# sunkafei/coffeedb

Measured on AMD Instinct MI355X. Metric: sa_build_GiB_per_s, higher is better.
Workload: dtype u64

## Files before the change

### coffeedb_amd/csrc/capi.hip

```cpp
#include <dirent.h>

#include <algorithm>
#include <chrono>
#include <condition_variable>
#include <cstdlib>
#include <cstring>
#include <thread>

#include "../../include/coffeedb_gpu.h"
#include "index_impl.h"

using namespace cdb;

namespace {

double wall_ms() {
    using namespace std::chrono;
    return duration<double, std::milli>(steady_clock::now().time_since_epoch()).count();
}

void set_error(Index& ix, const char* msg) {
    std::lock_guard<std::mutex> g(ix.err_mu);
    ix.err = msg;
}
// ... 1638 lines not shown
    else if (!std::strcmp(name, "reference_compat")) ix.reference_compat = value != 0;
    else if (!std::strcmp(name, "force_doubling")) ix.force_doubling = value != 0;
    else if (!std::strcmp(name, "initial_passes")) ix.initial_passes = (int)value;
    else if (!std::strcmp(name, "sort_variant")) ix.sort_variant = (int)value;
    else if (!std::strcmp(name, "keyhist3")) ix.keyhist3 = value != 0;
    else if (!std::strcmp(name, "key_symbols")) ix.key_symbols = (int)value;
    else if (!std::strcmp(name, "msd_first")) ix.msd_first = value != 0;
    else if (!std::strcmp(name, "msd_pair")) ix.msd_pair = value != 0;
    else if (!std::strcmp(name, "overlap_paircount")) ix.overlap_paircount = value != 0;
    else if (!std::strcmp(name, "key_directory")) { ix.key_directory = value != 0; ix.h_keydir.clear(); ix.keydir_tried = false; }
    else if (!std::strcmp(name, "fuse_records")) ix.fuse_records = value != 0;
    else if (!std::strcmp(name, "sweep_records")) ix.sweep_records = value != 0;
    else if (!std::strcmp(name, "partial_symbol")) ix.partial_symbol = value != 0;
    else if (!std::strcmp(name, "group_sort")) ix.group_sort = value != 0;
    else if (!std::strcmp(name, "list_rounds")) ix.list_rounds = value != 0;
    else if (!std::strcmp(name, "fuse_pairclass")) ix.fuse_pairclass = value != 0;
    else if (!std::strcmp(name, "group_sort_cap")) ix.group_sort_cap = (int)std::max<int64_t>(1, std::min<int64_t>(value, 1 << 20));
    else if (!std::strcmp(name, "vl_keys")) ix.vl_keys = value < 0 ? 0 : (value > 56 ? 56 : (int)value);
    else if (!std::strcmp(name, "pack_sa")) ix.pack_sa = value != 0;
    else if (!std::strcmp(name, "key_cost_model")) ix.key_cost_model = value != 0;
    else if (!std::strcmp(name, "gen_prebased")) ix.gen_prebased = value != 0;
    else if (!std::strcmp(name, "pack_entries")) ix.pack_entries = value != 0;
    else if (!std::strcmp(name, "segmented_sort")) ix.segmented_sort = value != 0;
    else if (!std::strcmp(name, "fold_root")) ix.fold_root = value != 0;
    else if (!std::strcmp(name, "fold_depth1")) ix.fold_depth1 = value != 0;
    else if (!std::strcmp(name, "flags_in_last_pass")) ix.flags_in_last_pass = value != 0;
    else if (!std::strcmp(name, "search_lanes")) ix.search_lanes = (value == 1 || value == 8) ? (int)value : 0;
    else if (!std::strcmp(name, "digit_bits")) ix.digit_bits = (int)value;
    else if (!std::strcmp(name, "fuse_keygen")) ix.fuse_keygen = value != 0;
    else if (!std::strcmp(name, "force_big_path")) ix.force_big_path = value != 0;
    else if (!std::strcmp(name, "debug_fail_build")) ix.debug_fail_build = value != 0;
    else if (!std::strcmp(name, "debug_append_path")) ix.debug_append_path = value == 1 || value == 2 ? (int)value : 0;
    else if (!std::strcmp(name, "debug_no_segcap")) ix.debug_no_segcap = value != 0;
    else if (!std::strcmp(name, "debug_starve_group")) ix.debug_starve_group = (int)value;
    else if (!std::strcmp(name, "self_check")) ix.self_check = value < 0 ? 0 : value > 3 ? 3 : (int)value;
    else if (!std::strcmp(name, "premap_generation")) ix.premap_generation = value != 0;
    else if (!std::strcmp(name, "proof_cancel")) {
        if (value) proof_stop(ix);
    }
    else if (!std::strcmp(name, "debug_damage_after_build")) ix.debug_damage_after_build = value < 0 ? 0 : (uint64_t)value;
    else if (!std::strcmp(name, "debug_fail_self_check")) ix.debug_fail_self_check = value != 0;
    else if (!std::strcmp(name, "plain_tile_order")) ix.rws.plain_order = value != 0;
    else if (!std::strcmp(name, "key_coding")) ix.key_coding = (int)value;
    else if (!std::strcmp(name, "narrow_keys")) ix.narrow_keys = value != 0;
    else if (!std::strcmp(name, "single_query")) ix.use_single_query = value != 0;
    else if (!std::strcmp(name, "resident_query")) {
// ... 5 lines not shown
    }
    else if (!std::strcmp(name, "bucket_group_limit")) ix.bucket_group_limit = (uint64_t)value;
    else if (!std::strcmp(name, "query_hit_budget"))
        ix.query_hit_budget = value > 0 ? std::min<uint64_t>((uint64_t)value, 1ull << 31) : 1;
    else if (!std::strcmp(name, "coalesce_queries")) ix.coalesce_queries = value != 0;
    else if (!std::strcmp(name, "fast_search")) ix.use_fast_search = value != 0;
    else if (!std::strcmp(name, "wave_rows")) ix.use_wave_rows = value != 0;
    else if (!std::strcmp(name, "keep_keys")) ix.keep_keys = value != 0;
    else {
        set_error(ix, (std::string("unknown option: ") + name).c_str());
        return CDB_E_INVALID;
    }
    return CDB_OK;
}

int cdb_get_stat(const cdb_index* h, const char* name, double* value) {
    if (!h || !name || !value) return CDB_E_INVALID;
    const BuildStats& b = h->ix.bstats;
    const QueryStats& q = h->ix.qstats;
    struct { const char* n; double v; } tab[] = {
        {"build_ms", b.build_ms}, {"alloc_ms", b.alloc_ms}, {"free_ms", b.free_ms}, {"rounds", (double)b.rounds}, {"ext_rounds", (double)b.ext_rounds},
        {"dbl_rounds", (double)b.dbl_rounds}, {"unresolved_after_initial", (double)b.unresolved_initial},
        {"unresolved_max", (double)b.unresolved_max}, {"sort_passes", (double)b.sort_passes},
        {"sort_passes_skipped", (double)b.sort_passes_skipped}, {"isa_built", (double)b.isa_built}, {"fused_keygen", (double)b.fused_keygen}, {"dense_keys", (double)b.dense_keys}, {"key_layout", (double)b.key_layout}, {"bucketed", (double)b.bucketed}, {"bucket_groups", (double)b.bucket_groups}, {"segmented", (double)b.segmented}, {"fused_records", (double)b.fused_records}, {"sweep_records", (double)b.sweep_records}, {"vl_key_bits", (double)b.vl_key_bits}, {"partial_levels", (double)b.partial_levels}, {"list_rounds", (double)b.list_rounds}, {"pairclass_fused", (double)b.pairclass_fused}, {"group_sorts", (double)b.group_sorts}, {"group_sort_fallbacks", (double)b.group_sort_fallbacks}, {"vl_avg_len", b.vl_avg_len}, {"vl_rate", b.vl_rate}, {"vl_est_unresolved", b.vl_est_unresolved}, {"fixed_est_unresolved", b.fixed_est_unresolved}, {"gen_prebased", (double)b.gen_prebased}, {"root_folded", (double)b.root_folded}, {"flags_in_last_pass", (double)b.flags_in_last_pass}, {"msd_first", (double)b.msd_first}, {"bucket_low_digits", (double)b.bucket_low_digits}, {"key_directory_cells", h->ix.h_keydir.empty() ? 0.0 : (double)(h->ix.h_keydir.size() - 1)}, {"group_fallbacks", (double)h->ix.group_fallbacks}, {"dense_key_retries", (double)h->ix.dense_key_retries}, {"self_check_fallbacks", (double)h->ix.self_check_fallbacks}, {"sa_packed", h->ix.sa_packed ? 1.0 : 0.0}, {"sa_bytes_per_entry", h->ix.sa_packed ? 5.0 : (double)h->ix.width}, {"self_check_pairs", (double)h->ix.self_check_pairs}, {"self_check_ms", h->ix.self_check_ms}, {"self_check_coverage", h->ix.size > 1 ? (double)h->ix.self_check_pairs / (double)(h->ix.size - 1) : 0.0},
        {"order_proved", (h->ix.proof.state.load() == 2 || h->ix.proof.state.load() == 3 || (h->ix.self_check == 2 && h->ix.width != 0)) ? 1.0 : 0.0},
        {"proof_state", (double)h->ix.proof.state.load()}, {"proof_ms", h->ix.proof.ms}, {"proof_repair_ms", h->ix.proof.repair_ms},
        {"proof_pairs", (double)h->ix.proof.pairs}, {"proof_bad_pairs", (double)h->ix.proof.found[0]}, {"proof_invalid_entries", (double)h->ix.proof.found[1]}, {"proof_skipped_pairs", (double)h->ix.proof.skipped}, {"proof_mixed_pairs", (double)h->ix.proof.mixed},
        {"proof_runs", (double)h->ix.proof.runs}, {"pool_big_mallocs", (double)DevPool::get().big_mallocs()}, {"premap_ms", h->ix.proof.premap_ms}, {"premap_bytes", (double)h->ix.proof.premap_bytes},
        {"key_symbols", (double)b.key_symbols}, {"symbol_bits", (double)b.symbol_bits},
        {"alphabet", (double)b.alphabet}, {"digit_bits", (double)b.digit_bits}, {"final_depth", (double)b.final_depth}, {"compat_rotations", (double)b.compat_rotations},
        {"compat_depth", (double)b.compat_depth},
        {"host_upload_ms", h->ix.host_upload_ms}, {"host_free_ms", h->ix.host_free_ms},
        {"resident_answers", (double)h->ix.res_answers}, {"launched_answers", (double)h->ix.launched_answers}, {"resident_mode", (double)h->ix.resident_mode},
        {"cluster_table_bytes", h->ix.clu.valid ? (double)(h->ix.clu.bytes() + h->ix.idt.bytes()) : 0.0}, {"cluster_classes", (double)h->ix.clu.nclasses},
        {"cluster_prepare_ms", h->ix.clu.prepare_ms}, {"cluster_ms", h->ix.clu.last_ms}, {"cluster_resorted", h->ix.clu.resorted ? 1.0 : 0.0},
        {"removes", (double)h->ix.rm.calls}, {"remove_compactions", (double)h->ix.rm.compactions}, {"remove_rebuilds", (double)h->ix.rm.rebuilds},
        {"remove_docs", (double)h->ix.rm.docs}, {"remove_bytes", (double)h->ix.rm.bytes}, {"remove_ms", h->ix.rm.last_ms},
        {"appends", (double)h->ix.ap.calls}, {"append_merges", (double)h->ix.ap.merges}, {"append_rebuilds", (double)h->ix.ap.rebuilds},
        {"append_docs", (double)h->ix.ap.docs}, {"append_bytes", (double)h->ix.ap.bytes}, {"append_ms", h->ix.ap.last_ms},
        {"append_keys_kept", (double)h->ix.ap.keys_kept},
        {"render_ms", h->ix.rnd.last_ms}, {"render_page_bytes", (double)h->ix.rnd.page_bytes}, {"render_spans", (double)h->ix.rnd.spans},
        {"query_ms", q.query_ms}, {"query_upload_ms", q.upload_ms}, {"query_device_ms", q.device_ms}, {"query_download_ms", q.download_ms}, {"query_hits", (double)q.nhits}, {"query_rows", (double)q.nrows},
        {"query_batches", (double)q.batches}, {"query_spec_batches", (double)q.spec_batches}, {"query_spec_spills", (double)q.spec_spills},
        {"query_wave_batches", (double)q.wave_batches}, {"query_sort_batches", (double)q.sort_batches}, {"query_sort_chunks", (double)q.sort_chunks},
        {"query_empty_batches", (double)q.empty_batches},
    };
    for (auto& e : tab)
// ... 204 lines not shown
```

### coffeedb_amd/csrc/index_impl.h

```cpp
#pragma once
#include <atomic>
#include <condition_variable>
#include <mutex>
#include <thread>
#include <string>
#include <vector>

#include "../../include/coffeedb_gpu.h"
#include "common.h"
#include "radix_sort.h"

namespace cdb {

constexpr int TEXT_PAD = 128;

struct BuildStats {
    double build_ms = 0, alloc_ms = 0, free_ms = 0;
    int rounds = 0;
    int ext_rounds = 0;
    int dbl_rounds = 0;
    uint64_t unresolved_initial = 0;
    uint64_t unresolved_max = 0;
    int sort_passes = 0;
    int sort_passes_skipped = 0;
    int isa_built = 0;
    int fused_keygen = 0;
    int key_layout = 0;
    int dense_keys = 0;
    int bucketed = 0;
    int bucket_low_digits = 0;
    int bucket_groups = 0;
    int root_folded = 0;
    int flags_in_last_pass = 0;
    int msd_first = 0;
    int gen_prebased = 0;
    int fused_records = 0;
    int sweep_records = 0;
    int pairclass_fused = 0;
    int list_rounds = 0;
    int group_sorts = 0, group_sort_fallbacks = 0;
    int partial_levels = 0;
    int vl_key_bits = 0;
    double vl_avg_len = 0, vl_rate = 0, vl_est_unresolved = 0, fixed_est_unresolved = 0;
    int segmented = 0;
    uint64_t gather_items = 0;
    int key_symbols = 0, symbol_bits = 0, alphabet = 0, digit_bits = 8;
    uint64_t final_depth = 0;
    uint64_t compat_rotations = 0, compat_depth = 0;
};

struct QueryStats {
    double query_ms = 0;
    double upload_ms = 0, device_ms = 0, download_ms = 0;
    uint64_t nhits = 0, nrows = 0;
    uint64_t batches = 0;
    uint64_t spec_batches = 0, spec_spills = 0;
    uint64_t wave_batches = 0;
    uint64_t sort_batches = 0, sort_chunks = 0;
    uint64_t empty_batches = 0;
};

struct SingleKeys {
    const uint64_t* keys64 = nullptr;
    const uint32_t* keys32 = nullptr;
    const void* keylow = nullptr;
    int low_bits = 0, low_bytes = 0, nsym = 0;
    bool decisive = false;
// ... 118 lines not shown
    int keydir_shift = 0, keydir_bits = 0;
    bool keydir_tried = false;
    bool key_directory = true;
    DevBuf d_pivots;
    int pivot_levels = 0;

    RadixWorkspace rws;
    MsdWorkspace msd_ws;
    DevBuf scan_partials;
    uint64_t q_spec_cap = 0;
    DevBuf q_spec;
    DevBuf q_pat, q_offs, q_left, q_right, q_hoff, q_keys0, q_keys1, q_flags, q_rowptr, q_ids, q_counts, q_hitptr, q_hitoff;

    bool reference_compat = true;
    bool force_doubling = false;
    int initial_passes = 0;
    int key_symbols = 0;
    int sort_variant = 0;
    int search_lanes = 0;
    bool flags_in_last_pass = true;
    bool fold_depth1 = true;
    bool fold_root = true;
    bool segmented_sort = true;
    bool fuse_records = true;
    bool fuse_pairclass = true;
    bool list_rounds = true;
    int group_sort_cap = 4096;
    bool group_sort = true;
    bool partial_symbol = true;
    int vl_keys = 2;
    bool vl_off_once = false;
    bool sweep_records = true;
    bool pack_entries = true;
    bool msd_first = true;
    bool msd_pair = true;
    bool keyhist3 = true;
    int dense_key_retries = 0;
    int group_fallbacks = 0;
    uint64_t bucket_group_limit = 0;
    uint64_t self_check_pairs = 0;
    double self_check_ms = 0;
    int self_check = 3;
    int self_check_fallbacks = 0;
    bool debug_fail_self_check = false;
    struct Proof {
        std::thread th;
// ... 254 lines not shown
```

### coffeedb_amd/csrc/radix_sort.h

```cpp
#pragma once
#include <cstdlib>

#include "common.h"

namespace cdb {

constexpr int RS_MAX_PASSES = 16;

constexpr uint64_t RS_VAL_MASK = (1ull << 54) - 1;
constexpr uint32_t RS_SPIN_LIMIT_GROUPED = 1u << 18;
constexpr uint32_t RS_SPIN_LIMIT_PLAIN = 1u << 22;
constexpr int RS_GROUP = 8;

struct NoVal {};

template <typename K, typename V> struct RsTraits { static constexpr int IPT = 12; };
template <> struct RsTraits<uint64_t, uint32_t> { static constexpr int IPT = 15; };
template <> struct RsTraits<uint64_t, uint64_t> { static constexpr int IPT = 12; };

template <typename K>
__global__ __launch_bounds__(256) void rs_hist_kernel(const K* __restrict__ keys, uint64_t n, int begin_bit,
                                                      int npass, int dbits, uint32_t last_mask,
                                                      unsigned long long* __restrict__ ghist) {
    __shared__ uint32_t sh[RS_MAX_PASSES * 256];
// ... 150 lines not shown
    return r < si.rot_b ? slot + (len - si.rot_b) : slot - (si.rot_b - si.rot_a);
}
struct SegArgs {
    const uint32_t* tile_seg = nullptr;
    const SegInfo* segs = nullptr;
    uint32_t tiles = 0;
    uint32_t start_stride = 0;
};
struct SegEdge {
    unsigned long long first, last;
    unsigned long long pos;
    uint32_t cnt, pad;
};
struct SegFinalArgs : SegArgs {
    uint64_t* eout = nullptr;
    uint32_t* elo = nullptr;
    uint8_t* ehi = nullptr;
    uint8_t* flags = nullptr;
    SegEdge* edges = nullptr;
    int hi_shift = 0;
    int low_bits = 0;
    uint32_t kbase = 2;
    unsigned long long kmagic = 0;
};

struct SegFinalKeepArgs : SegArgs {
    uint8_t* flags = nullptr;
    SegEdge* edges = nullptr;
    int low_bits = 0;
    uint32_t kbase = 2;
    unsigned long long kmagic = 0;
    unsigned long long* tile_sums = nullptr;
    uint32_t sums_tile = 1;
    unsigned long long msd_m = 0;
};

struct SegFinalKeepMsdArgs : SegFinalKeepArgs {};

__device__ __forceinline__ uint64_t rs_pack_key(const uint32_t* __restrict__ s_words, uint32_t li, int nsym, uint32_t base,
                                                uint32_t rem) {
    const uint32_t wi = li >> 2, sel = li & 3u;
    const uint32_t b2 = base * base, b3 = b2 * base;
    const uint32_t pw[5] = {1u, base, b2, b3, b3 * base};
    uint64_t kk = 0;
    uint32_t lo = s_words[wi];
#pragma unroll
    for (int w = 0; w < 4; ++w) {
// ... 19 lines not shown
        const uint64_t mid = lo + (hi - lo + 1) / 2;
        if (doc_start[mid] <= p) lo = mid; else hi = mid - 1;
    }
    return lo;
}

static __global__ __launch_bounds__(256) void rs_tiledoc_kernel(const uint64_t* __restrict__ doc_start, uint64_t ndocs,
                                                                uint64_t n, uint64_t tile_elems, uint64_t tiles,
                                                                uint64_t* __restrict__ tile_doc) {
    const uint64_t t = (uint64_t)blockIdx.x * 256 + threadIdx.x;
    if (t > tiles) return;
    const uint64_t p = t * tile_elems < n ? t * tile_elems : n - 1;
    tile_doc[t] = rs_doc_upper(doc_start, 0, ndocs - 1, p);
}

template <typename K, typename V, typename Cfg, typename Gen = NoGen, typename W = NoVal, typename Seg = NoSeg>
__global__ __launch_bounds__(Cfg::NT, Cfg::MINW) void rs_onesweep_kernel(
    const K* __restrict__ kin, K* __restrict__ kout, const V* __restrict__ vin, V* __restrict__ vout, uint64_t n,
    int shift, uint32_t dmask, const unsigned long long* __restrict__ digit_start, uint64_t* __restrict__ status,
    uint32_t* __restrict__ ticket, uint32_t epoch, uint32_t* __restrict__ err, Gen gen = Gen(),
    const W* __restrict__ win = nullptr, W* __restrict__ wout = nullptr, int aux_shift = -1, Seg seg = Seg()) {
    constexpr bool GEN = !std::is_same<Gen, NoGen>::value;
    constexpr bool SEG = !std::is_same<Seg, NoSeg>::value;
    constexpr bool FINAL = std::is_same<Seg, SegFinalArgs>::value;
    constexpr bool KEEPM = std::is_same<Seg, SegFinalKeepMsdArgs>::value;
    constexpr bool KEEP = std::is_same<Seg, SegFinalKeepArgs>::value || KEEPM;
    constexpr bool FLAGS = FINAL || KEEP;
    static_assert(!SEG || (!GEN && !Cfg::DMA), "segmented passes: materialised records");
    static_assert(!FLAGS || Cfg::REUSE || KEEPM, "flag-writing passes: shared staging (the MSD-first last pass also runs with keys and values staged at once)");
    constexpr bool HAS_V = !std::is_same<V, NoVal>::value;
    constexpr bool HAS_W = !std::is_same<W, NoVal>::value;
    using WS = typename std::conditional<HAS_W, W, uint8_t>::type;
    static_assert(!HAS_W || KEEPM || (Cfg::REUSE && HAS_V && !Cfg::DMA), "the auxiliary byte needs the shared-staging configuration");
    constexpr int IPT = Cfg::IPT;
    constexpr bool REUSE = Cfg::REUSE && HAS_V;
    constexpr bool EARLYV = (Cfg::EARLYV || REUSE) && HAS_V;
    constexpr int NT = Cfg::NT;
    constexpr int NW = NT / 64;
    constexpr bool NTM = Cfg::NONTEMP;
    constexpr int TILE = NT * IPT;
    constexpr int WCHUNK = 64 * IPT;
    using VS = typename std::conditional<HAS_V, V, uint32_t>::type;
    constexpr size_t STAGE_K = sizeof(K) * TILE;
    constexpr size_t STAGE_V = HAS_V ? sizeof(VS) * TILE : 0;
    constexpr size_t STAGE_BYTES = REUSE ? (STAGE_K > STAGE_V ? STAGE_K : STAGE_V) : STAGE_K + STAGE_V;

    constexpr bool BLK = GEN && sizeof(K) == 4 && sizeof(VS) == 4 && IPT == 16 && (NT == 1024 || NT == 512);
// ... 631 lines not shown
                    const uint64_t kf = ktop + (uint64_t)k;
                    uint32_t f = head ? 1u : 0u;
                    if (!(head && tail)) {
                        const bool exhausted = seg.kmagic ? (kf - __umul64hi(kf, seg.kmagic) * seg.kbase) == 0
                                                          : (kf & (uint64_t)(seg.kbase - 1u)) == 0;
                        if (!exhausted) f |= 2u;
                    }
                    seg.flags[dst] = (uint8_t)f;
                    if ((f & 2u) && seg.tile_sums) {
                        atomicAdd(seg.tile_sums + 2 * (dst / seg.sums_tile), 1ull);
                        if (f & 1u) atomicAdd(seg.tile_sums + 2 * (dst / seg.sums_tile) + 1, 1ull);
                    }
                    rs_store<NTM>(kout + dst, (K)(kf >> 8));
                    if constexpr (HAS_W) rs_store<NTM>(wout + dst, (W)(kf & 0xFFu));
                    rs_store<NTM>(vout + dst, (V)s_vals[i]);
                    continue;
                }
                if (!GEN || kout) rs_store<NTM>(kout + dst, k);
                if constexpr (HAS_V) rs_store<NTM>(vout + dst, (V)s_vals[i]);
            }
        }
    } else {
        uint8_t dig[IPT];
#pragma unroll
        for (int j = 0; j < IPT; ++j) {
            const uint32_t i = j * NT + tid;
            dig[j] = 0;
            if (i < valid) {
                const K k = s_keys[i];
                uint32_t dd;
                if constexpr (KEEPM) dd = (uint32_t)(k >> shift) & dmask;
                else dd = digit_of(k, s_aux[HAS_W ? i : 0]);
                if constexpr (recs) dd = (uint32_t)s_gen[i];
                dig[j] = (uint8_t)dd;
                if constexpr (FLAGS) {
                    const uint32_t lmask = seg.low_bits >= 32 ? 0xFFFFFFFFu : (1u << seg.low_bits) - 1u;
                    uint32_t ac = 0;
                    if constexpr (!KEEPM) ac = (uint32_t)s_aux[HAS_W ? i : 0] & lmask;
                    bool head = true, tail = true;
                    bool cmp = true;
                    if constexpr (FINAL) cmp = !(RS_SEG_ABL & 4);
                    if constexpr (KEEPM) {
                        if (i > 0) head = s_keys[i - 1] != k;
                        if (i + 1 < valid) tail = s_keys[i + 1] != k;
                    } else if (cmp) {
                        if (i > 0) head = s_keys[i - 1] != k || ((uint32_t)s_aux[HAS_W ? i - 1 : 0] & lmask) != ac;
                        if (i + 1 < valid) tail = s_keys[i + 1] != k || ((uint32_t)s_aux[HAS_W ? i + 1 : 0] & lmask) != ac;
                    }
                    uint32_t f = head ? 1u : 0u;
                    if (!(head && tail)) {
                        const uint64_t kc = KEEPM ? ktop + (uint64_t)k : (((uint64_t)k << seg.low_bits) | (uint64_t)ac);
                        const bool exhausted = seg.kmagic ? (kc - __umul64hi(kc, seg.kmagic) * seg.kbase) == 0
                                                          : (kc & (uint64_t)(seg.kbase - 1u)) == 0;
                        if (!exhausted) f |= 2u;
                    }
                    if constexpr (FINAL) {
                        if (!(RS_SEG_ABL & 1)) seg.flags[rs_seg_rotated(si, s_gbase[dd] + i)] = (uint8_t)f;
                        continue;
                    } else {
                        const uint64_t slot = s_gbase[dd] + i;
                        seg.flags[slot] = (uint8_t)f;
                        if ((f & 2u) && seg.tile_sums) {
                            atomicAdd(seg.tile_sums + 2 * (slot / seg.sums_tile), 1ull);
                            if (f & 1u) atomicAdd(seg.tile_sums + 2 * (slot / seg.sums_tile) + 1, 1ull);
                        }
                    }
                }
                if constexpr (KEEPM) {
                    const uint64_t kf = ktop + (uint64_t)k;
                    rs_store<NTM>(kout + s_gbase[dd] + i, (K)(kf >> 8));
                    if constexpr (HAS_W) rs_store<NTM>(wout + s_gbase[dd] + i, (W)(kf & 0xFFu));
                    continue;
                }
                if (!GEN || kout) rs_store<NTM>(kout + s_gbase[dd] + i, k);
                if constexpr (HAS_W && !W32G) {
                    if (!GEN || wout) rs_store<NTM>(wout + s_gbase[dd] + i, (W)s_aux[i]);
                }
            }
        }
        __syncthreads();
        if constexpr (W32G) {
#pragma unroll
            for (int j = 0; j < IPT; ++j) s_vals[rank[j]] = (VS)aux[j];
            __syncthreads();
#pragma unroll
            for (int j = 0; j < IPT; ++j) {
                const uint32_t i = j * NT + tid;
                if (i < valid) rs_store<NTM>(wout + s_gbase[dig[j]] + i, (W)s_vals[i]);
            }
            __syncthreads();
        }
#pragma unroll
        for (int j = 0; j < IPT; ++j) s_vals[rank[j]] = val[j];
        __syncthreads();
#pragma unroll
        for (int j = 0; j < IPT; ++j) {
            const uint32_t i = j * NT + tid;
            if constexpr (FINAL) {
                if (i < valid && !(RS_SEG_ABL & 2)) {
                    const unsigned long long slot = rs_seg_rotated(si, s_gbase[dig[j]] + i);
                    const uint32_t hi32 = (uint32_t)s_aux[HAS_W ? i : 0] >> seg.hi_shift;
                    if (seg.elo) {
                        seg.elo[slot] = (uint32_t)s_vals[i];
                        seg.ehi[slot] = (uint8_t)hi32;
                    } else {
                        seg.eout[slot] = ((uint64_t)hi32 << 32) | (uint64_t)s_vals[i];
                    }
                }
            } else {
                if constexpr (GEN && sizeof(VS) == 8) {
                    if (gen.vout_hi) {
                        if (i < valid) {
                            const uint64_t dst = s_gbase[dig[j]] + i;
                            const uint64_t e = (uint64_t)s_vals[i];
                            reinterpret_cast<uint32_t*>(vout)[dst] = (uint32_t)e;
                            gen.vout_hi[dst] = (uint8_t)(e >> 32);
                        }
                        continue;
                    }
                }
                if (i < valid) rs_store<NTM>(vout + s_gbase[dig[j]] + i, (V)s_vals[i]);
            }
        }
    }
}

static __global__ __launch_bounds__(256) void rs_seg_edge_fix_kernel(const SegEdge* __restrict__ edges, const uint32_t* __restrict__ tile_seg,
                                                                     const SegInfo* __restrict__ segs, uint32_t tiles,
                                                                     uint8_t* __restrict__ flags, uint32_t kbase, unsigned long long kmagic,
                                                                     unsigned long long* __restrict__ tile_sums = nullptr,
                                                                     uint32_t sums_tile = 1, const uint32_t* __restrict__ err = nullptr) {
    const uint32_t t = blockIdx.x, d = threadIdx.x;
    if (t >= tiles) return;
    if (err && *err) return;
    const SegEdge e = edges[(size_t)t * 256 + d];
    if (!e.cnt) return;
    const SegInfo si = segs[tile_seg ? tile_seg[t] : 0u];
    const uint32_t t0 = si.tile_begin;
    if (t == t0) return;
    uint32_t lo = t0, hi = t;
    if (edges[(size_t)(t - 1) * 256 + d].pos < e.pos) {
        lo = t - 1;
    } else {
        if (edges[(size_t)t0 * 256 + d].pos >= e.pos) return;
        hi = t - 1;
        while (hi - lo > 1) {
            const uint32_t mid = lo + (hi - lo) / 2;
            if (edges[(size_t)mid * 256 + d].pos < e.pos) lo = mid; else hi = mid;
        }
    }
    const SegEdge pe = edges[(size_t)lo * 256 + d];
    if (pe.last != e.first) return;
    const bool exhausted = kmagic ? (e.first - __umul64hi(e.first, kmagic) * kbase) == 0 : (e.first & (uint64_t)(kbase - 1u)) == 0;
    auto change = [&](unsigned long long slot, uint32_t clear, uint32_t set) {
        const uintptr_t a = reinterpret_cast<uintptr_t>(flags + slot);
        unsigned int* w = reinterpret_cast<unsigned int*>(a & ~(uintptr_t)3);
        const uint32_t sh = 8u * (uint32_t)(a & 3u);
        uint32_t before, after;
        if (clear) {
            before = (atomicAnd(w, ~(clear << sh)) >> sh) & 0xFFu;
            after = before & ~clear;
        } else {
            before = (atomicOr(w, set << sh) >> sh) & 0xFFu;
            after = before | set;
        }
        if (tile_sums && before != after) {
            const long long da = (long long)((after >> 1) & 1u) - (long long)((before >> 1) & 1u);
            const long long db = (long long)((after >> 1) & after & 1u) - (long long)((before >> 1) & before & 1u);
            unsigned long long* ts = tile_sums + 2 * (slot / sums_tile);
            if (da) atomicAdd(ts, (unsigned long long)da);
            if (db) atomicAdd(ts + 1, (unsigned long long)db);
        }
    };
    const unsigned long long sb = rs_seg_rotated(si, e.pos), sa_ = rs_seg_rotated(si, e.pos - 1);
    change(sb, 1u, 0u);
    if (!exhausted) {
        change(sb, 0u, 2u);
        change(sa_, 0u, 2u);
    }
}

static __global__ __launch_bounds__(256) void rs_lane_order_probe_kernel(uint32_t* __restrict__ bad) {
    __shared__ uint32_t cnt[4][256];
    __shared__ uint32_t ref[4][256];
    const int tid = threadIdx.x, lane = tid & 63, wave = tid >> 6;
    for (int i = tid; i < 4 * 256; i += 256) {
        (&cnt[0][0])[i] = 0;
        (&ref[0][0])[i] = 0;
    }
    __syncthreads();
    const uint64_t lt_mask = (1ull << lane) - 1ull;
    uint32_t wrong = 0;
// ... 415 lines not shown
    __shared__ unsigned long long s[256];
    const uint32_t g = blockIdx.x;
    const int t = threadIdx.x;
    const unsigned long long b0 = segs[g].begin;
    for (int p = 0; p < npass; ++p) {
        const unsigned long long c = hist[((size_t)g * 8 + p) * 256 + t];
        s[t] = c;
        __syncthreads();
        for (int off = 1; off < 256; off <<= 1) {
            const unsigned long long v = t >= off ? s[t - off] : 0;
            __syncthreads();
            s[t] += v;
            __syncthreads();
        }
        starts[((size_t)g * 8 + p) * 256 + t] = b0 + s[t] - c;
        __syncthreads();
    }
}

template <typename W>
void radix_sort_segmented(hipStream_t s, RadixWorkspace& ws, Profiler& prof, uint32_t* k0, uint32_t* k1, uint32_t* v0, uint32_t* v1,
                          W* w0, W* w1, uint64_t m, const SegInfo* d_segs, const uint32_t* d_tile_seg, uint32_t nseg, uint32_t tiles,
                          const unsigned long long* d_hist, unsigned long long* d_starts, int key_bits, int lead, SegFinalArgs fin,
                          SortStats* stats) {
    if (!rs_atomic_rank_ok(s)) throw Error("radix_sort_segmented: needs the one-atomic ranking (internal)");
    const int kpass = (int)ceil_div((uint64_t)key_bits, 8);
    const int npass = kpass + lead;
    if (npass < 1 || npass > 8 || kpass < 1) throw Error("radix_sort_segmented: unsupported pass count (internal)");
    const int last_bits = key_bits - 8 * (kpass - 1);
    const uint32_t last_mask = (1u << last_bits) - 1u;
    ws.prepare((uint64_t)tiles * RS_SEG_TILE, RS_SEG_TILE, s);
    hipLaunchKernelGGL(rs_seg_digit_start_kernel, dim3(nseg), dim3(256), 0, s, d_hist, d_segs, npass, d_starts);
    SegArgs sa;
    sa.tile_seg = d_tile_seg;
    sa.segs = d_segs;
    sa.tiles = tiles;
    sa.start_stride = 8 * 256;
    static_cast<SegArgs&>(fin) = sa;
    const bool grouped = ws.allow_group && !ws.plain_order;
    using CfgG = RsCfg<16, true, true, 1024, false, 1, 0, 4, false, true, true, 1, RS_GROUP>;
    using CfgP = RsCfg<16, true, true, 1024, false, 1, 0, 4, false, true>;
    const uint32_t grid = grouped ? (uint32_t)(ceil_div(tiles, 8u * RS_GROUP) * 8u * RS_GROUP) : tiles;
    uint32_t* kb[2] = {k0, k1};
    uint32_t* vb[2] = {v0, v1};
    W* wb[2] = {w0, w1};
    int cur = 0;
    const char* wn = sizeof(W) == 1 ? "_w8" : (sizeof(W) == 2 ? "_w16" : "_w32");
    const size_t rec = 8 + sizeof(W);
    for (int p = 0; p < npass; ++p) {
        const uint32_t e = ws.next_epoch(s);
        const uint32_t dmask = p == npass - 1 ? last_mask : 0xFFu;
        const int shift = 8 * (p - lead);
        const int aux_shift = p < lead ? 8 * p : -1;
        const unsigned long long* dstart = d_starts + (size_t)p * 256;
        uint32_t* tk = grouped ? ws.xticket_ptr(e) : ws.ticket_ptr(e);
        int t = prof.begin(s);
#define CDB_SEG_LAUNCH(CFG, SEGT, SEGV)                                                                                       \
    hipLaunchKernelGGL((rs_onesweep_kernel<uint32_t, uint32_t, CFG, NoGen, W, SEGT>), dim3(grid), dim3(1024), 0, s,            \
                       (const uint32_t*)kb[cur], kb[cur ^ 1], (const uint32_t*)vb[cur], vb[cur ^ 1], m, shift, dmask, dstart, \
                       ws.status.as<uint64_t>(), tk, e, ws.err_ptr(), NoGen(), (const W*)wb[cur], wb[cur ^ 1], aux_shift,     \
                       SEGV)
        if (p == npass - 1) {
            if (grouped) CDB_SEG_LAUNCH(CfgG, SegFinalArgs, fin);
            else CDB_SEG_LAUNCH(CfgP, SegFinalArgs, fin);
            prof.end(t, (std::string("rs_seg_final") + wn + "_t16384").c_str(), m * (rec + (fin.elo ? 6 : 9)), s);
        } else {
            if (grouped) CDB_SEG_LAUNCH(CfgG, SegArgs, sa);
            else CDB_SEG_LAUNCH(CfgP, SegArgs, sa);
            prof.end(t, (std::string("rs_seg_k32_v32") + wn + "_t16384").c_str(), 2 * m * rec, s);
        }
#undef CDB_SEG_LAUNCH
        cur ^= 1;
        if (stats) stats->passes_run++;
    }
    int t = prof.begin(s);
    hipLaunchKernelGGL(rs_seg_edge_fix_kernel, dim3(tiles), dim3(256), 0, s, (const SegEdge*)fin.edges, d_tile_seg, d_segs, tiles,
                       fin.flags, fin.kbase, fin.kmagic, (unsigned long long*)nullptr, 1u, (const uint32_t*)ws.err_ptr());
    prof.end(t, "rs_seg_edge_fix", (uint64_t)tiles * 256 * sizeof(SegEdge), s);
    CDB_HIP(hipGetLastError());
}

constexpr int RS_MSD_HIST_TILES = 32;

template <typename W>
__global__ __launch_bounds__(1024) void rs_seg_hist_kernel(const uint32_t* __restrict__ keys, const W* __restrict__ aux, int lead, int npass,
                                                           const uint32_t* __restrict__ tile_seg, const SegInfo* __restrict__ segs,
                                                           uint32_t tiles, unsigned long long* __restrict__ hist) {
    constexpr int NC = 4, HC = 8 * 256 + 64 / NC;
    __shared__ uint32_t sh4[NC * HC];
    const int tid = threadIdx.x;
    uint32_t* const sh = sh4 + (tid & (NC - 1)) * HC;
    const uint32_t t0 = blockIdx.x * RS_MSD_HIST_TILES;
    const uint32_t t1 = t0 + RS_MSD_HIST_TILES < tiles ? t0 + RS_MSD_HIST_TILES : tiles;
    uint32_t cur = ~0u;
    auto flush = [&]() {
        __syncthreads();
        if (cur != ~0u)
            for (int i = tid; i < npass * 256; i += 1024) {
                uint32_t c = 0;
#pragma unroll
// ... 411 lines not shown
```

### coffeedb_amd/csrc/records_sweep.h

```cpp
#pragma once
#include "radix_sort.h"

namespace cdb {

#ifndef RS_SWEEP_ABL
#define RS_SWEEP_ABL 0
#endif
#ifndef RS_SWEEP_UNALIGNED
#define RS_SWEEP_UNALIGNED 0
#endif
__device__ __forceinline__ int rs_uniform(int x) {
    int y = __builtin_amdgcn_readfirstlane(x);
    asm volatile("" : "+s"(y));
    return y;
}
__device__ __forceinline__ uint32_t rs_wave_incl_scan(uint32_t x) {
    uint32_t v = x;
    v += (uint32_t)__builtin_amdgcn_update_dpp(0, (int)x, 0x111, 0xf, 0xf, false);
    v += (uint32_t)__builtin_amdgcn_update_dpp(0, (int)x, 0x112, 0xf, 0xf, false);
    v += (uint32_t)__builtin_amdgcn_update_dpp(0, (int)x, 0x113, 0xf, 0xf, false);
    v += (uint32_t)__builtin_amdgcn_update_dpp(0, (int)v, 0x114, 0xf, 0xe, false);
    v += (uint32_t)__builtin_amdgcn_update_dpp(0, (int)v, 0x118, 0xf, 0xc, false);
    v += (uint32_t)__builtin_amdgcn_update_dpp(0, (int)v, 0x142, 0xa, 0xf, false);
    v += (uint32_t)__builtin_amdgcn_update_dpp(0, (int)v, 0x143, 0xc, 0xf, false);
    return v;
}

constexpr int RS_SWEEP_TILE = RS_GEN8_TILE;
constexpr uint32_t RS_SWEEP_DOCS = 768;

template <typename W>
__global__ __launch_bounds__(512, 8) void rs_sweep_records_kernel(TextGen gen, const uint16_t* __restrict__ codeslot, uint64_t n, uint32_t tiles,
                                                                  uint32_t g0, uint32_t g1, uint64_t gstart, uint32_t* __restrict__ kout,
                                                                  uint32_t* __restrict__ vout, W* __restrict__ wout) {
    constexpr int NT = 512, IPT = 16, TILE = RS_SWEEP_TILE, NW = NT / 64;
    static_assert(NT * IPT == TILE, "tile shape");
    constexpr int abl = RS_SWEEP_ABL;
    constexpr uint32_t TEXTB = ((TILE + RS_GEN_LOOK + 15) / 16) * 16;
// ... 835 lines not shown
```

### coffeedb_amd/csrc/sa_build.hip

```cpp
#include <algorithm>
#include <chrono>
#include <cmath>
#include <cstdlib>
#include <cstring>

#include "index_impl.h"
#include "records_sweep.h"
#include "vl_code.h"
#include "scan.h"

#ifndef RS_GATHER_ABL
#define RS_GATHER_ABL 0
#endif

namespace cdb {
namespace {

constexpr int KG_TILE = 2048;
constexpr int KG_LOOK = 64;

__global__ __launch_bounds__(256) void sa_bytecount_kernel(const uint8_t* __restrict__ text, uint64_t n,
                                                           unsigned long long* __restrict__ counts) {
    __shared__ uint32_t s[256];
    s[threadIdx.x] = 0;
// ... 2530 lines not shown
                }
                wb[q] = std::move(rf.fr_w[q]);
                continue;
            } else {
                kb[q].alloc(max_elems * sizeof(uint32_t));
                eb[q].alloc(max_elems * sizeof(uint32_t));
                kbp[q] = kb[q].as<uint32_t>();
                ebp[q] = eb[q].as<uint32_t>();
            }
            wb[q].alloc(max_elems * sizeof(W));
        }
        edges.alloc((size_t)max_tiles * 256 * sizeof(SegEdge));
        d_starts.alloc((size_t)max_gb * 8 * 256 * sizeof(uint64_t));
        d_bh2.alloc((size_t)max_gb * 8 * 256 * sizeof(uint64_t));
        d_segs.alloc((size_t)nb * sizeof(SegInfo));
        tile_seg.alloc((size_t)max_tiles * sizeof(uint32_t));
        cell_off.alloc((size_t)max_cells * sizeof(uint32_t));
        lists.alloc(groups.size() * 16 * sizeof(uint32_t));
        d_items2.alloc((size_t)max_items * sizeof(BucketItem));
        st.alloc_ms += now_ms() - ta;
        CDB_HIP(hipMemcpyAsync(d_segs.p, h_segs.data(), (size_t)nb * sizeof(SegInfo), hipMemcpyHostToDevice, s));
        CDB_HIP(hipMemsetAsync(lists.p, 0, groups.size() * 16 * sizeof(uint32_t), s));
        const unsigned long long* bnd = br.d_bounds.as<unsigned long long>();
        for (size_t gi = 0; gi < groups.size(); ++gi) {
            const Group& g = groups[gi];
            const uint32_t gb = g.b1 - g.b0;
            uint32_t* list_len = lists.as<uint32_t>() + gi * 16;
            uint32_t* tickets = list_len + 8;
            if (fuse_rec && !sweep_fused) {
                {
                    hipLaunchKernelGGL(rs_seg_tilemap_kernel, dim3((unsigned)ceil_div(g.tiles, 256)), dim3(256), 0, s,
                                       (const SegInfo*)(d_segs.as<SegInfo>() + g.b0), gb, g.tiles, tile_seg.as<uint32_t>());
                    TextGen rg{text, doc_start, al.d_symmap.as<uint16_t>(), D, (int)ix.bits, bbase, nsym, 0, ix.text_padded};
                    rg.slotmap = d_slotmap.as<uint8_t>();
                    rg.rec_low_bits = blow;
                    radix_gen_records<W>(s, ix.rws, ix.prof, kbp[0], ebp[0], wb[0].as<W>(), n,
                                         bk.first_digit.data(), rg, (const uint32_t*)tile_seg.as<uint32_t>(),
                                         (const SegInfo*)(d_segs.as<SegInfo>() + g.b0), gb, g.tiles, lowb, bpass,
                                         d_bh2.as<unsigned long long>(), &ss,
                                         tile_bytes ? (const uint32_t*)al.d_tbc.as<uint32_t>() : nullptr,
                                         tile_bytes ? (const uint16_t*)bk.d_src_col.as<uint16_t>() : nullptr, tile_bytes ? &ix.tbw : nullptr);
                    st.gen_prebased = tile_bytes ? 1 : 0;
                }
            } else if (sweep_rec || sweep_fused) {
                hipLaunchKernelGGL(rs_seg_tilemap_kernel, dim3((unsigned)ceil_div(g.tiles, 256)), dim3(256), 0, s,
                                   (const SegInfo*)(d_segs.as<SegInfo>() + g.b0), gb, g.tiles, tile_seg.as<uint32_t>());
// ... 45 lines not shown
                               (const uint16_t*)al.d_symmap.as<uint16_t>(), (int)ix.bits, ix.mask, nsym, bbase, blow, bpass, g.gstart,
                               g.b0, kbp[0], wb[0].as<W>(), ebp[0], d_bh2.as<unsigned long long>());
            ix.prof.end(t, "sa_bucket_records", g.elems * ((uint64_t)nsym + recb + sizeof(V)), s);
            st.gather_items += g.elems / BR_ITEM;
            hipLaunchKernelGGL(rs_seg_tilemap_kernel, dim3((unsigned)ceil_div(g.tiles, 256)), dim3(256), 0, s,
                               (const SegInfo*)(d_segs.as<SegInfo>() + g.b0), gb, g.tiles, tile_seg.as<uint32_t>());
            }
            SegFinalArgs fin;
            if (pack_seg) {
                fin.elo = E.as<uint32_t>() + g.gstart;
                fin.ehi = out.sa_hi_buf.as<uint8_t>() + g.gstart;
            } else if (out.packed_out) {
                fin.elo = kbp[dead] + g.gstart;
                fin.ehi = out.sa_hi_buf.as<uint8_t>() + g.gstart;
            } else {
                fin.eout = (fuse_rec ? kb[dead].as<uint64_t>() : E.as<uint64_t>()) + g.gstart;
            }
            fin.flags = out.flags.as<uint8_t>() + g.gstart;
            fin.edges = edges.as<SegEdge>();
            fin.hi_shift = blow;
            fin.low_bits = blow;
            fin.kbase = br.fbase;
            fin.kmagic = br.bmagic;
            radix_sort_segmented<W>(s, ix.rws, ix.prof, kbp[0], kbp[1], ebp[0], ebp[1], wb[0].as<W>(), wb[1].as<W>(), g.elems,
                                    (const SegInfo*)(d_segs.as<SegInfo>() + g.b0), (const uint32_t*)tile_seg.as<uint32_t>(), gb,
                                    g.tiles, (const unsigned long long*)d_bh2.as<unsigned long long>(),
                                    d_starts.as<unsigned long long>(), rf.bbits - blow, lowb, fin, &ss);
            st.bucket_groups++;
        }
        CDB_HIP(hipStreamSynchronize(s));
        if (sweep_rec || sweep_fused) ix.tbw.base.release();
        if (fuse_rec) E = std::move(kb[dead]);
        if (pack_seg) out.packed_out = true;
        st.segmented = 1;
    }
}

template <typename V, typename I>
void run_per_bucket(Index& ix, const Alphabet& al, const KeyPlan& kp, const Buckets& bk, const RecordForm& rf, const BucketRecords& br,
                    DevBuf& E, InitialSort& out, SortStats& ss) {
    hipStream_t s = ix.stream;
    const uint64_t n = ix.size;
    BuildStats& st = ix.bstats;
    const uint8_t* text = ix.d_text;
    const uint64_t* doc_start = ix.d_doc_start.as<uint64_t>();
    const int nsym = kp.nsym;
    const uint32_t nb = br.nb, nch = br.nch, bbase = rf.bbase;
    const std::vector<uint64_t>& bstart = br.bstart;
    const int bbits = rf.bbits, blow = rf.blow, bpass = br.bpass, lowb = br.lowb, keyb = br.keyb, auxb = br.auxb, recb = br.recb;
    const bool packed = rf.packed;
    const uint64_t maxb = bk.maxb, bmagic = br.bmagic;
    const double avail = br.avail;
    std::vector<uint64_t> bounds((size_t)nb * (nch + 1));
    CDB_HIP(hipMemcpyAsync(bounds.data(), br.d_bounds.p, bounds.size() * 8, hipMemcpyDeviceToHost, s));
    CDB_HIP(hipStreamSynchronize(s));
    const bool third = !packed && avail > (double)maxb * (2.0 * (keyb + lowb) + 2 * sizeof(V)) * 1.15;
    const double scratch = packed ? (double)maxb * recb
// ... 787 lines not shown
```

Baseline: 30.09.

## Add one-phase segmented final radix pass writing flags and entries together

```diff
diff --git a/coffeedb_amd/csrc/capi.hip b/coffeedb_amd/csrc/capi.hip
--- a/coffeedb_amd/csrc/capi.hip
+++ b/coffeedb_amd/csrc/capi.hip
@@ -1684,6 +1684,7 @@
     else if (!std::strcmp(name, "gen_prebased")) ix.gen_prebased = value != 0;
     else if (!std::strcmp(name, "pack_entries")) ix.pack_entries = value != 0;
     else if (!std::strcmp(name, "segmented_sort")) ix.segmented_sort = value != 0;
+    else if (!std::strcmp(name, "seg_final_one_phase")) ix.seg_final_one_phase = value == 0 || value == 1 ? (int)value : 2;
     else if (!std::strcmp(name, "fold_root")) ix.fold_root = value != 0;
     else if (!std::strcmp(name, "fold_depth1")) ix.fold_depth1 = value != 0;
     else if (!std::strcmp(name, "flags_in_last_pass")) ix.flags_in_last_pass = value != 0;
@@ -1735,7 +1736,7 @@
         {"build_ms", b.build_ms}, {"alloc_ms", b.alloc_ms}, {"free_ms", b.free_ms}, {"rounds", (double)b.rounds}, {"ext_rounds", (double)b.ext_rounds},
         {"dbl_rounds", (double)b.dbl_rounds}, {"unresolved_after_initial", (double)b.unresolved_initial},
         {"unresolved_max", (double)b.unresolved_max}, {"sort_passes", (double)b.sort_passes},
-        {"sort_passes_skipped", (double)b.sort_passes_skipped}, {"isa_built", (double)b.isa_built}, {"fused_keygen", (double)b.fused_keygen}, {"dense_keys", (double)b.dense_keys}, {"key_layout", (double)b.key_layout}, {"bucketed", (double)b.bucketed}, {"bucket_groups", (double)b.bucket_groups}, {"segmented", (double)b.segmented}, {"fused_records", (double)b.fused_records}, {"sweep_records", (double)b.sweep_records}, {"vl_key_bits", (double)b.vl_key_bits}, {"partial_levels", (double)b.partial_levels}, {"list_rounds", (double)b.list_rounds}, {"pairclass_fused", (double)b.pairclass_fused}, {"group_sorts", (double)b.group_sorts}, {"group_sort_fallbacks", (double)b.group_sort_fallbacks}, {"vl_avg_len", b.vl_avg_len}, {"vl_rate", b.vl_rate}, {"vl_est_unresolved", b.vl_est_unresolved}, {"fixed_est_unresolved", b.fixed_est_unresolved}, {"gen_prebased", (double)b.gen_prebased}, {"root_folded", (double)b.root_folded}, {"flags_in_last_pass", (double)b.flags_in_last_pass}, {"msd_first", (double)b.msd_first}, {"bucket_low_digits", (double)b.bucket_low_digits}, {"key_directory_cells", h->ix.h_keydir.empty() ? 0.0 : (double)(h->ix.h_keydir.size() - 1)}, {"group_fallbacks", (double)h->ix.group_fallbacks}, {"dense_key_retries", (double)h->ix.dense_key_retries}, {"self_check_fallbacks", (double)h->ix.self_check_fallbacks}, {"sa_packed", h->ix.sa_packed ? 1.0 : 0.0}, {"sa_bytes_per_entry", h->ix.sa_packed ? 5.0 : (double)h->ix.width}, {"self_check_pairs", (double)h->ix.self_check_pairs}, {"self_check_ms", h->ix.self_check_ms}, {"self_check_coverage", h->ix.size > 1 ? (double)h->ix.self_check_pairs / (double)(h->ix.size - 1) : 0.0},
+        {"sort_passes_skipped", (double)b.sort_passes_skipped}, {"isa_built", (double)b.isa_built}, {"fused_keygen", (double)b.fused_keygen}, {"dense_keys", (double)b.dense_keys}, {"key_layout", (double)b.key_layout}, {"bucketed", (double)b.bucketed}, {"bucket_groups", (double)b.bucket_groups}, {"segmented", (double)b.segmented}, {"seg_final_one_phase", (double)b.seg_final_one_phase}, {"fused_records", (double)b.fused_records}, {"sweep_records", (double)b.sweep_records}, {"vl_key_bits", (double)b.vl_key_bits}, {"partial_levels", (double)b.partial_levels}, {"list_rounds", (double)b.list_rounds}, {"pairclass_fused", (double)b.pairclass_fused}, {"group_sorts", (double)b.group_sorts}, {"group_sort_fallbacks", (double)b.group_sort_fallbacks}, {"vl_avg_len", b.vl_avg_len}, {"vl_rate", b.vl_rate}, {"vl_est_unresolved", b.vl_est_unresolved}, {"fixed_est_unresolved", b.fixed_est_unresolved}, {"gen_prebased", (double)b.gen_prebased}, {"root_folded", (double)b.root_folded}, {"flags_in_last_pass", (double)b.flags_in_last_pass}, {"msd_first", (double)b.msd_first}, {"bucket_low_digits", (double)b.bucket_low_digits}, {"key_directory_cells", h->ix.h_keydir.empty() ? 0.0 : (double)(h->ix.h_keydir.size() - 1)}, {"group_fallbacks", (double)h->ix.group_fallbacks}, {"dense_key_retries", (double)h->ix.dense_key_retries}, {"self_check_fallbacks", (double)h->ix.self_check_fallbacks}, {"sa_packed", h->ix.sa_packed ? 1.0 : 0.0}, {"sa_bytes_per_entry", h->ix.sa_packed ? 5.0 : (double)h->ix.width}, {"self_check_pairs", (double)h->ix.self_check_pairs}, {"self_check_ms", h->ix.self_check_ms}, {"self_check_coverage", h->ix.size > 1 ? (double)h->ix.self_check_pairs / (double)(h->ix.size - 1) : 0.0},
         {"order_proved", (h->ix.proof.state.load() == 2 || h->ix.proof.state.load() == 3 || (h->ix.self_check == 2 && h->ix.width != 0)) ? 1.0 : 0.0},
         {"proof_state", (double)h->ix.proof.state.load()}, {"proof_ms", h->ix.proof.ms}, {"proof_repair_ms", h->ix.proof.repair_ms},
         {"proof_pairs", (double)h->ix.proof.pairs}, {"proof_bad_pairs", (double)h->ix.proof.found[0]}, {"proof_invalid_entries", (double)h->ix.proof.found[1]}, {"proof_skipped_pairs", (double)h->ix.proof.skipped}, {"proof_mixed_pairs", (double)h->ix.proof.mixed},
diff --git a/coffeedb_amd/csrc/index_impl.h b/coffeedb_amd/csrc/index_impl.h
--- a/coffeedb_amd/csrc/index_impl.h
+++ b/coffeedb_amd/csrc/index_impl.h
@@ -43,6 +43,7 @@
     int vl_key_bits = 0;
     double vl_avg_len = 0, vl_rate = 0, vl_est_unresolved = 0, fixed_est_unresolved = 0;
     int segmented = 0;
+    int seg_final_one_phase = 0;
     uint64_t gather_items = 0;
     int key_symbols = 0, symbol_bits = 0, alphabet = 0, digit_bits = 8;
     uint64_t final_depth = 0;
@@ -207,6 +208,7 @@
     bool fold_depth1 = true;
     bool fold_root = true;
     bool segmented_sort = true;
+    int seg_final_one_phase = 2;
     bool fuse_records = true;
     bool fuse_pairclass = true;
     bool list_rounds = true;
diff --git a/coffeedb_amd/csrc/radix_sort.h b/coffeedb_amd/csrc/radix_sort.h
--- a/coffeedb_amd/csrc/radix_sort.h
+++ b/coffeedb_amd/csrc/radix_sort.h
@@ -196,7 +196,21 @@
     int low_bits = 0;
     uint32_t kbase = 2;
     unsigned long long kmagic = 0;
+    unsigned long long* tile_sums = nullptr;
+    uint32_t sums_tile = 1;
+    unsigned long long sums_base = 0;
 };
+struct SegFinalOneArgs : SegFinalArgs {};
+
+__device__ __forceinline__ int rs_uniform(int x) {
+    int y = __builtin_amdgcn_readfirstlane(x);
+    asm volatile("" : "+s"(y));
+    return y;
+}
+__device__ __forceinline__ unsigned long long rs_uniform64(unsigned long long x) {
+    const uint32_t lo = (uint32_t)rs_uniform((int)(uint32_t)x), hi = (uint32_t)rs_uniform((int)(uint32_t)(x >> 32));
+    return ((unsigned long long)hi << 32) | lo;
+}
 
 struct SegFinalKeepArgs : SegArgs {
     uint8_t* flags = nullptr;
@@ -262,7 +276,8 @@
     const W* __restrict__ win = nullptr, W* __restrict__ wout = nullptr, int aux_shift = -1, Seg seg = Seg()) {
     constexpr bool GEN = !std::is_same<Gen, NoGen>::value;
     constexpr bool SEG = !std::is_same<Seg, NoSeg>::value;
-    constexpr bool FINAL = std::is_same<Seg, SegFinalArgs>::value;
+    constexpr bool FINAL1 = std::is_same<Seg, SegFinalOneArgs>::value;
+    constexpr bool FINAL = std::is_same<Seg, SegFinalArgs>::value || FINAL1;
     constexpr bool KEEPM = std::is_same<Seg, SegFinalKeepMsdArgs>::value;
     constexpr bool KEEP = std::is_same<Seg, SegFinalKeepArgs>::value || KEEPM;
     constexpr bool FLAGS = FINAL || KEEP;
@@ -940,6 +955,8 @@
         }
     } else {
         uint8_t dig[IPT];
+        uint32_t fl = 0;
+        static_assert(!FINAL1 || IPT <= 16, "one-phase final pass: 2 flag bits per record in one register");
 #pragma unroll
         for (int j = 0; j < IPT; ++j) {
             const uint32_t i = j * NT + tid;
@@ -972,7 +989,10 @@
                                                           : (kc & (uint64_t)(seg.kbase - 1u)) == 0;
                         if (!exhausted) f |= 2u;
                     }
-                    if constexpr (FINAL) {
+                    if constexpr (FINAL1) {
+                        fl |= f << (2 * j);
+                        continue;
+                    } else if constexpr (FINAL) {
                         if (!(RS_SEG_ABL & 1)) seg.flags[rs_seg_rotated(si, s_gbase[dd] + i)] = (uint8_t)f;
                         continue;
                     } else {
@@ -1011,6 +1031,36 @@
 #pragma unroll
         for (int j = 0; j < IPT; ++j) s_vals[rank[j]] = val[j];
         __syncthreads();
+        if constexpr (FINAL1) {
+            const int sums_shift = __builtin_ctz(seg.sums_tile);
+            auto emit = [&](auto rotated, unsigned long long ra, unsigned long long rb, unsigned long long sbeg, unsigned long long slen) {
+#pragma unroll
+                for (int j = 0; j < IPT; ++j) {
+                    const uint32_t i = j * NT + tid;
+                    if (i < valid) {
+                        unsigned long long slot = s_gbase[dig[j]] + i;
+                        if constexpr (decltype(rotated)::value) {
+                            const unsigned long long r = slot - sbeg;
+                            if (r >= ra) slot = r < rb ? slot + (slen - rb) : slot - (rb - ra);
+                        }
+                        const uint32_t f = (fl >> (2 * j)) & 3u;
+                        seg.flags[slot] = (uint8_t)f;
+                        seg.elo[slot] = (uint32_t)s_vals[i];
+                        seg.ehi[slot] = (uint8_t)((uint32_t)s_aux[HAS_W ? i : 0] >> seg.hi_shift);
+                        if ((f & 2u) && seg.tile_sums) {
+                            unsigned long long* ts = seg.tile_sums + 2 * ((seg.sums_base + slot) >> sums_shift);
+                            atomicAdd(ts, 1ull);
+                            if (f & 1u) atomicAdd(ts + 1, 1ull);
+                        }
+                    }
+                }
+            };
+            if (rs_uniform(si.rot_b != 0 ? 1 : 0))
+                emit(std::true_type{}, rs_uniform64(si.rot_a), rs_uniform64(si.rot_b), rs_uniform64(si.begin), rs_uniform64(si.end - si.begin));
+            else
+                emit(std::false_type{}, 0ull, 0ull, 0ull, 0ull);
+            return;
+        }
 #pragma unroll
         for (int j = 0; j < IPT; ++j) {
             const uint32_t i = j * NT + tid;
@@ -1047,7 +1097,8 @@
                                                                      const SegInfo* __restrict__ segs, uint32_t tiles,
                                                                      uint8_t* __restrict__ flags, uint32_t kbase, unsigned long long kmagic,
                                                                      unsigned long long* __restrict__ tile_sums = nullptr,
-                                                                     uint32_t sums_tile = 1, const uint32_t* __restrict__ err = nullptr) {
+                                                                     uint32_t sums_tile = 1, const uint32_t* __restrict__ err = nullptr,
+                                                                     unsigned long long sums_base = 0) {
     const uint32_t t = blockIdx.x, d = threadIdx.x;
     if (t >= tiles) return;
     if (err && *err) return;
@@ -1085,7 +1136,7 @@
         if (tile_sums && before != after) {
             const long long da = (long long)((after >> 1) & 1u) - (long long)((before >> 1) & 1u);
             const long long db = (long long)((after >> 1) & after & 1u) - (long long)((before >> 1) & before & 1u);
-            unsigned long long* ts = tile_sums + 2 * (slot / sums_tile);
+            unsigned long long* ts = tile_sums + 2 * ((sums_base + slot) / sums_tile);
             if (da) atomicAdd(ts, (unsigned long long)da);
             if (db) atomicAdd(ts + 1, (unsigned long long)db);
         }
@@ -1547,7 +1598,10 @@
 void radix_sort_segmented(hipStream_t s, RadixWorkspace& ws, Profiler& prof, uint32_t* k0, uint32_t* k1, uint32_t* v0, uint32_t* v1,
                           W* w0, W* w1, uint64_t m, const SegInfo* d_segs, const uint32_t* d_tile_seg, uint32_t nseg, uint32_t tiles,
                           const unsigned long long* d_hist, unsigned long long* d_starts, int key_bits, int lead, SegFinalArgs fin,
-                          SortStats* stats) {
+                          SortStats* stats, bool one_phase = false) {
+    if (one_phase && (!fin.elo || !fin.ehi || RS_SEG_ABL)) throw Error("radix_sort_segmented: one-phase final pass needs packed entries (internal)");
+    if (!one_phase) fin.tile_sums = nullptr;
+    if (fin.tile_sums && (fin.sums_tile == 0 || (fin.sums_tile & (fin.sums_tile - 1)))) throw Error("radix_sort_segmented: scan tiles must be a power of two (internal)");
     if (!rs_atomic_rank_ok(s)) throw Error("radix_sort_segmented: needs the one-atomic ranking (internal)");
     const int kpass = (int)ceil_div((uint64_t)key_bits, 8);
     const int npass = kpass + lead;
@@ -1586,8 +1640,15 @@
                        ws.status.as<uint64_t>(), tk, e, ws.err_ptr(), NoGen(), (const W*)wb[cur], wb[cur ^ 1], aux_shift,     \
                        SEGV)
         if (p == npass - 1) {
-            if (grouped) CDB_SEG_LAUNCH(CfgG, SegFinalArgs, fin);
-            else CDB_SEG_LAUNCH(CfgP, SegFinalArgs, fin);
+            if (one_phase) {
+                SegFinalOneArgs fin1;
+                static_cast<SegFinalArgs&>(fin1) = fin;
+                if (grouped) CDB_SEG_LAUNCH(CfgG, SegFinalOneArgs, fin1);
+                else CDB_SEG_LAUNCH(CfgP, SegFinalOneArgs, fin1);
+            } else {
+                if (grouped) CDB_SEG_LAUNCH(CfgG, SegFinalArgs, fin);
+                else CDB_SEG_LAUNCH(CfgP, SegFinalArgs, fin);
+            }
             prof.end(t, (std::string("rs_seg_final") + wn + "_t16384").c_str(), m * (rec + (fin.elo ? 6 : 9)), s);
         } else {
             if (grouped) CDB_SEG_LAUNCH(CfgG, SegArgs, sa);
@@ -1600,7 +1661,8 @@
     }
     int t = prof.begin(s);
     hipLaunchKernelGGL(rs_seg_edge_fix_kernel, dim3(tiles), dim3(256), 0, s, (const SegEdge*)fin.edges, d_tile_seg, d_segs, tiles,
-                       fin.flags, fin.kbase, fin.kmagic, (unsigned long long*)nullptr, 1u, (const uint32_t*)ws.err_ptr());
+                       fin.flags, fin.kbase, fin.kmagic, fin.tile_sums, fin.tile_sums ? fin.sums_tile : 1u, (const uint32_t*)ws.err_ptr(),
+                       fin.sums_base);
     prof.end(t, "rs_seg_edge_fix", (uint64_t)tiles * 256 * sizeof(SegEdge), s);
     CDB_HIP(hipGetLastError());
 }
diff --git a/coffeedb_amd/csrc/records_sweep.h b/coffeedb_amd/csrc/records_sweep.h
--- a/coffeedb_amd/csrc/records_sweep.h
+++ b/coffeedb_amd/csrc/records_sweep.h
@@ -9,11 +9,6 @@
 #ifndef RS_SWEEP_UNALIGNED
 #define RS_SWEEP_UNALIGNED 0
 #endif
-__device__ __forceinline__ int rs_uniform(int x) {
-    int y = __builtin_amdgcn_readfirstlane(x);
-    asm volatile("" : "+s"(y));
-    return y;
-}
 __device__ __forceinline__ uint32_t rs_wave_incl_scan(uint32_t x) {
     uint32_t v = x;
     v += (uint32_t)__builtin_amdgcn_update_dpp(0, (int)x, 0x111, 0xf, 0xf, false);
diff --git a/coffeedb_amd/csrc/sa_build.hip b/coffeedb_amd/csrc/sa_build.hip
--- a/coffeedb_amd/csrc/sa_build.hip
+++ b/coffeedb_amd/csrc/sa_build.hip
@@ -2576,6 +2576,13 @@
         CDB_HIP(hipMemcpyAsync(d_segs.p, h_segs.data(), (size_t)nb * sizeof(SegInfo), hipMemcpyHostToDevice, s));
         CDB_HIP(hipMemsetAsync(lists.p, 0, groups.size() * 16 * sizeof(uint32_t), s));
         const unsigned long long* bnd = br.d_bounds.as<unsigned long long>();
+        const bool one_phase = ix.seg_final_one_phase && (pack_seg || out.packed_out) && !RS_SEG_ABL;
+        const bool counted = one_phase && ix.seg_final_one_phase == 1;
+        if (counted) {
+            const uint64_t nbt = ceil_div(n, (uint64_t)SC_TILE);
+            ix.scan_partials.ensure(scan_partials_slots(nbt) * sizeof(U2));
+            CDB_HIP(hipMemsetAsync(ix.scan_partials.p, 0, nbt * sizeof(U2), s));
+        }
         for (size_t gi = 0; gi < groups.size(); ++gi) {
             const Group& g = groups[gi];
             const uint32_t gb = g.b1 - g.b0;
@@ -2667,10 +2674,15 @@
             fin.low_bits = blow;
             fin.kbase = br.fbase;
             fin.kmagic = br.bmagic;
+            if (counted) {
+                fin.tile_sums = ix.scan_partials.as<unsigned long long>();
+                fin.sums_tile = SC_TILE;
+                fin.sums_base = g.gstart;
+            }
             radix_sort_segmented<W>(s, ix.rws, ix.prof, kbp[0], kbp[1], ebp[0], ebp[1], wb[0].as<W>(), wb[1].as<W>(), g.elems,
                                     (const SegInfo*)(d_segs.as<SegInfo>() + g.b0), (const uint32_t*)tile_seg.as<uint32_t>(), gb,
                                     g.tiles, (const unsigned long long*)d_bh2.as<unsigned long long>(),
-                                    d_starts.as<unsigned long long>(), rf.bbits - blow, lowb, fin, &ss);
+                                    d_starts.as<unsigned long long>(), rf.bbits - blow, lowb, fin, &ss, one_phase);
             st.bucket_groups++;
         }
         CDB_HIP(hipStreamSynchronize(s));
@@ -2678,6 +2690,8 @@
         if (fuse_rec) E = std::move(kb[dead]);
         if (pack_seg) out.packed_out = true;
         st.segmented = 1;
+        st.seg_final_one_phase = one_phase ? ix.seg_final_one_phase : 0;
+        out.tile_sums_ready = counted;
     }
 }
 
```

New measurement: 29.90. No clear change (-0.6%).
